# JuliaDSP/DSP.jl

Measured on NVIDIA H100. Metric: Gsamples/s filt+welch on 2^26 cplx-F32, higher is better.
Workload: dtype c64 (ComplexF32; f32 arithmetic)

## Files before the change

### __graft_entry__.py

```python
import os
import subprocess
import sys

ROOT = os.path.dirname(os.path.abspath(__file__))
PKG = os.path.join(ROOT, "dsp.jl_b200")


def build() -> None:
    jobs = str(min(8, os.cpu_count() or 2))
    subprocess.run(["make", "-C", os.path.join(PKG, "csrc"), "-j", jobs], check=True)
    host_dir = os.path.join(ROOT, "tests", "host")
    os.makedirs(os.path.join(ROOT, "build"), exist_ok=True)
    for name in ("fft_core_host_check", "fft_r32_host_check"):
        subprocess.run(["g++", "-std=c++17", "-O2", "-x", "c++", "-w", "-I/usr/local/cuda/include",
                        "-o", os.path.join(ROOT, "build", name), os.path.join(host_dir, name + ".cu")], check=True)
    for name in ("fir_tile_host_check", "fir_state_host_check"):
        subprocess.run(["g++", "-std=c++17", "-O2", "-march=native", "-x", "c++", "-w", "-I/usr/local/cuda/include",
                        "-o", os.path.join(ROOT, "build", name), os.path.join(host_dir, name + ".cu")], check=True)
    if ROOT not in sys.path:
        sys.path.insert(0, ROOT)
    import dspb200
    assert dspb200._lib.lib.dspb200_version() == 100


def smoke() -> None:
    if ROOT not in sys.path:
        sys.path.insert(0, ROOT)
    import numpy as np
    import dspb200
    from oracle import dspbase as od, periodograms as op, windows as ow

    if dspb200.device_count() < 1:
        raise RuntimeError("smoke() needs a CUDA device; dspb200 has no CPU fallback")
    rng = np.random.default_rng(7)
    x = (rng.standard_normal(1 << 16) + 1j * rng.standard_normal(1 << 16)).astype(np.complex64)
    v = (rng.standard_normal(513) + 1j * rng.standard_normal(513)).astype(np.complex64)
    y = dspb200.conv(x, v, algorithm="fft_overlapsave")
    ref = od.conv_exact(x, v)
    err = np.linalg.norm(y - ref) / np.linalg.norm(ref)
    assert y.dtype == np.complex64 and err < 1e-6, f"conv parity {err}"
    s = rng.standard_normal(1 << 18).astype(np.float32)
    p = dspb200.welch_pgram(s, 4096, 2048, window=dspb200.hanning)
    pref, _ = op.welch_pgram(s, 4096, 2048, window=ow.hanning, f64=True)
    err2 = np.linalg.norm(p.power - pref) / np.linalg.norm(pref)
    assert p.power.dtype == np.float32 and err2 < 1e-6, f"welch parity {err2}"
    print(f"smoke ok: conv relerr {err:.2e}, welch relerr {err2:.2e}, launches {dspb200.launch_count()}")


if __name__ == "__main__":
    build()
    if len(sys.argv) > 1 and sys.argv[1] == "smoke":
        smoke()
```

### dsp.jl_b200/csrc/fft_core.cuh

```cuda
#pragma once
#include "common.cuh"
#include <math.h>

#ifndef DSP_PROBE
#define DSP_PROBE 0
#endif

namespace dspb200 {

template <typename T> struct fft_pad { static constexpr int K = sizeof(T) == 4 ? 2 : 1; };
template <typename T> __host__ __device__ constexpr int fft_pad256(int n) {
    if (sizeof(T) == 4) return n == 512 ? 8 : (n == 1024 ? 4 : (n == 8192 ? 4 : 2));
    return n == 512 ? 4 : (n == 1024 ? 2 : (n == 8192 ? 2 : 1));
}
template <typename T> __host__ __device__ constexpr int fft_pad4096(int n) {
    if (sizeof(T) == 4) return n == 8192 ? 2 : (n == 16384 ? 4 : 0);
    return n == 8192 ? 1 : 0;
}
template <typename T, int N> __host__ __device__ __forceinline__ constexpr int padaddr(int p) {
    return p + fft_pad<T>::K * (p >> 4) + fft_pad256<T>(N) * (p >> 8) + fft_pad4096<T>(N) * (p >> 12);
}
template <typename T> __host__ __device__ constexpr int padded_len(int n) {
    return ((n - 1) + fft_pad<T>::K * ((n - 1) >> 4) + fft_pad256<T>(n) * ((n - 1) >> 8) + fft_pad4096<T>(n) * ((n - 1) >> 12) + 1 + 3) & ~3;
}
// ... 335 lines not shown
        fft_bfly<T, 16, false>(v0, w0);
#pragma unroll
        for (int r = 0; r < 16; ++r) p0[r * PS] = v0[r];
        fft_bfly<T, 16, false>(v1, w1);
#pragma unroll
        for (int r = 0; r < 16; ++r) p1[r * PS] = v1[r];
        return;
    }
#pragma unroll 1
    for (int it = 0; it < ITERS; ++it) {
        const int b = tid + it * NT;
        if (Q % NT != 0 && b >= Q) break;
        const int t = b & (S - 1);
        cx<T>* p = c.sm + padaddr<T, N>((b / S) * (16 * S) + t);
        cx<T> v[16], w[8];
        if constexpr (GATE && ITERS == 1) fft_gate_wait<NT>(tid);
        load_tw8<T, S, fft_tw_row(N)>(tab, t, w);
#pragma unroll
        for (int r = 0; r < 16; ++r) v[r] = p[r * PS];
        if constexpr (GATE && ITERS == 1) fft_gate_open<NT>(tid);
        fft_bfly<T, 16, false>(v, w);
#pragma unroll
        for (int r = 0; r < 16; ++r) p[r * PS] = v[r];
    }
}

template <typename T, int N, int NT, class Scope = FftCtaScope>
__device__ __forceinline__ void fft_middle(const FftCtx<T>& c, int tid, Scope sc = Scope()) {
    constexpr int NMID = fft_plan_traits<N>::NMID;
    static_assert(NMID < 2 || std::is_same<Scope, FftCtaScope>::value, "thread groups run transforms of at most 4096 points");
    if constexpr (NMID >= 1) {
#if !(DSP_PROBE & 16)
        fft_pass16<T, N, NT, 16, true>(c, tid);
#endif
        if constexpr (NMID == 2) {
            fft_group256_sync<NT>(tid);
#if !(DSP_PROBE & 1)
            fft_pass16<T, N, NT, 256>(c, tid);
#endif
        }
        sc.sync();
    }
}

template <typename T, int N>
__host__ __device__ __forceinline__ void fft_last_pass_load(const FftCtx<T>& c, int tp, cx<T> (&v)[16]) {
    constexpr int Q = fft_plan_traits<N>::Q;
    const cx<T>* p = c.sm + padaddr<T, N>(tp);
#pragma unroll
    for (int r = 0; r < 16; ++r) v[r] = p[padaddr<T, N>(r * Q)];
}
template <typename T, int N>
__host__ __device__ __forceinline__ void fft_last_pass_bfly(const FftCtx<T>& c, int tp, cx<T> (&v)[16]) {
    using P = fft_plan_traits<N>;
    constexpr int Q = P::Q, RL = P::RL;
    if constexpr (RL == 16) {
        cx<T> w[8];
        load_tw8<T, Q, fft_tw_row(N)>(Q == 16 ? c.t16 : c.t256, tp, w);
        fft_bfly<T, 16, false>(v, w);
    } else {
        constexpr int NBF = 16 / RL;
        constexpr int TLK = P::TLK;
#pragma unroll
        for (int a = 0; a < NBF; ++a) {
            const int t = tp + Q * a;
            cx<T> w[RL / 2];
            if constexpr (N == 16384) {
                const cx<T> w1 = fft_tl_in_smem<T, N>() ? c.tl[t] : ldtw<T>(c.tl, t);
                w[1] = w1;
                w[0] = mkc<T>(fma_(w1.x, w1.x, -(w1.y * w1.y)), (w1.x + w1.x) * w1.y);
            } else {
#pragma unroll
                for (int i = 0; i < TLK; ++i) w[i] = fft_tl_in_smem<T, N>() ? c.tl[t * TLK + i] : ldtw<T>(c.tl, t * TLK + i);
            }
            cx<T> u[RL];
#pragma unroll
            for (int j = 0; j < RL; ++j) u[j] = v[a + NBF * j];
            fft_bfly<T, RL, false>(u, w);
#pragma unroll
            for (int j = 0; j < RL; ++j) v[a + NBF * j] = u[j];
        }
    }
}
template <typename T, int N, int GATE_NT = 0>
__host__ __device__ __forceinline__ void fft_last_pass(const FftCtx<T>& c, int tp, cx<T> (&v)[16], int tid = 0) {
    if constexpr (GATE_NT > 256) fft_gate_wait<GATE_NT>(tid);
    fft_last_pass_load<T, N>(c, tp, v);
    if constexpr (GATE_NT > 256) fft_gate_open<GATE_NT>(tid);
    fft_last_pass_bfly<T, N>(c, tp, v);
}

template <int N> struct fft_last_chunks {
    static constexpr int RL = fft_plan_traits<N>::RL;
    static constexpr int COUNT = 16 / RL;
};
template <typename T, int N, int A>
__device__ __forceinline__ void fft_last_pass_chunk(const FftCtx<T>& c, int tp, cx<T> (&u)[fft_plan_traits<N>::RL]) {
    using P = fft_plan_traits<N>;
    constexpr int Q = P::Q, RL = P::RL, NBF = 16 / RL;
    const cx<T>* p = c.sm + padaddr<T, N>(tp);
#pragma unroll
    for (int j = 0; j < RL; ++j) u[j] = p[padaddr<T, N>((A + NBF * j) * Q)];
    if constexpr (RL == 16) {
        cx<T> w[8];
        load_tw8<T, Q, fft_tw_row(N)>(Q == 16 ? c.t16 : c.t256, tp, w);
        fft_bfly<T, 16, false>(u, w);
    } else {
        const int t = tp + Q * A;
        cx<T> w[RL / 2];
        if constexpr (N == 16384) {
            const cx<T> w1 = fft_tl_in_smem<T, N>() ? c.tl[t] : ldtw<T>(c.tl, t);
            w[1] = w1;
            w[0] = mkc<T>(fma_(w1.x, w1.x, -(w1.y * w1.y)), (w1.x + w1.x) * w1.y);
        } else {
#pragma unroll
            for (int i = 0; i < P::TLK; ++i) w[i] = fft_tl_in_smem<T, N>() ? c.tl[t * P::TLK + i] : ldtw<T>(c.tl, t * P::TLK + i);
        }
        fft_bfly<T, RL, false>(u, w);
    }
}

template <typename T, int N, int NT, class Ld0, class StLast>
__device__ __forceinline__ void fft_forward(const FftCtx<T>& c, int tid, Ld0 ld0, StLast stlast) {
    constexpr int Q = fft_plan_traits<N>::Q;
    constexpr int ITERS = (Q + NT - 1) / NT;
    fft_first_pass<T, N, NT, false>(c, tid, ld0);
    __syncthreads();
    fft_middle<T, N, NT>(c, tid);
#pragma unroll
    for (int it = 0; it < ITERS; ++it) {
        const int tp = tid + it * NT;
        if (Q % NT != 0 && tp >= Q) break;
        cx<T> v[16];
        fft_last_pass<T, N>(c, tp, v);
#pragma unroll
        for (int r = 0; r < 16; ++r) stlast(tp + r * Q, it, r, v[r]);
    }
}

struct fft_r32 {
    static constexpr int N = 16384;
    static constexpr int NT = 512;
    static constexpr int Q = N / 32;
    static constexpr int QL = N / 16;
    static constexpr int T32_LEN = 32 * 16;
    static constexpr int TL_LEN = 2 * QL;
    static constexpr int TABLE_LEN = T32_LEN + TL_LEN;
    static constexpr int C10 = 2;
    static constexpr int PADDED_LEN = ((N - 1) + C10 * ((N - 1) >> 10) + 1 + 3) & ~3;
    static constexpr int SMEM_ELEMS = PADDED_LEN + TABLE_LEN;
};
__host__ __device__ __forceinline__ constexpr int fft_r32_padaddr(int p) { return p + fft_r32::C10 * (p >> 10); }
__host__ __device__ __forceinline__ constexpr int fft_r32_block_of(int c) { return 32 * (c & 15) + (c >> 4); }

template <typename T> struct FftR32Ctx {
    cx<T>* sm;
    const cx<T>* t32;
    const cx<T>* tl;
};
template <typename T>
__device__ __forceinline__ FftR32Ctx<T> fft_r32_make_ctx(cx<T>* data, cx<T>* tabs, const cx<T>* __restrict__ g, int tid) {
    for (int i = tid; i < fft_r32::TABLE_LEN; i += fft_r32::NT) tabs[i] = g[i];
    return FftR32Ctx<T>{data, tabs, tabs + fft_r32::T32_LEN};
}

template <typename T> __host__ __device__ __forceinline__ void fft_r32_first_bfly(cx<T> (&v)[32]) { fft_bfly<T, 32, true>(v, nullptr); }
template <typename T> __host__ __device__ __forceinline__ void fft_r32_store_block(cx<T>* sm, int c, const cx<T> (&v)[32]) {
    cx<T>* p = sm + fft_r32_padaddr(32 * fft_r32_block_of(c));
#pragma unroll
    for (int r = 0; r < 32; r += 2) sts2<T>(p + r, v[r], v[r + 1]);
}

template <typename T, bool GATE = false> __host__ __device__ __forceinline__ void fft_r32_middle(const FftR32Ctx<T>& c, int tid) {
    const int t = tid & 31;
    cx<T>* p = c.sm + fft_r32_padaddr((tid >> 5) * 1024 + t);
    cx<T> v[32], w[16];
    if constexpr (GATE) fft_gate_wait<fft_r32::NT>(tid);
#pragma unroll
    for (int i = 0; i < 16; i += 2) lds2<T>(c.t32 + fft_tw_index<T>(i, t, 32), w[i], w[i + 1]);
#pragma unroll
    for (int r = 0; r < 32; ++r) v[r] = p[32 * r];
    if constexpr (GATE) fft_gate_open<fft_r32::NT>(tid);
    fft_bfly<T, 32, false>(v, w);
#pragma unroll
    for (int r = 0; r < 32; ++r) p[32 * r] = v[r];
}

template <typename T> __host__ __device__ __forceinline__ void fft_r32_last_load(const FftR32Ctx<T>& c, int t, cx<T> (&v)[16]) {
    const cx<T>* p = c.sm + fft_r32_padaddr(t);
#pragma unroll
    for (int s = 0; s < 16; ++s) v[s] = p[fft_r32_padaddr(s * 1024)];
}
template <typename T> __host__ __device__ __forceinline__ cx<T> fft_sq(cx<T> a) {
    return mkc<T>(fma_(a.x, a.x, -(a.y * a.y)), (a.x + a.x) * a.y);
}
template <typename T> __host__ __device__ __forceinline__ cx<T> fft_mul_const(cx<T> a, T cr, T ci) {
    return mkc<T>(fma_(a.x, cr, -(a.y * ci)), fma_(a.x, ci, a.y * cr));
}
template <typename T> __host__ __device__ __forceinline__ void fft_r32_last_bfly(const FftR32Ctx<T>& c, int t, cx<T> (&v)[16]) {
    const T c16 = fft_const<T>::C8, s16 = fft_const<T>::S8;
    cx<T> w[8];
    lds2<T>(c.tl + 2 * t, w[1], w[4]);
    w[2] = fft_sq(w[4]);
    w[0] = fft_sq(w[1]);
    w[3] = mul_w8<T>(w[2]);
    w[5] = fft_mul_const<T>(w[4], c16, -s16);
    w[6] = mul_w8<T>(w[4]);
    w[7] = fft_mul_const<T>(w[4], s16, -c16);
    fft_bfly<T, 16, false>(v, w);
}

template <typename T> inline void fft_fill_row(cx<T>* row, int R, long long num, long long den, int limit = 1 << 30) {
    const long double PI2 = 6.283185307179586476925286766559005768L;
    int qb = 0;
    for (int r = R; r > 1; r >>= 1) ++qb;
    int idx = 0;
    for (int k = 1; k <= qb; ++k) {
        const int cnt = k <= 2 ? 1 : (1 << (k - 2));
        for (int m = 0; m < cnt; ++m) {
            const long double a = -PI2 * ((long double)num * (long double)(R >> k) / (long double)den + (long double)m / (long double)(1 << k));
            if (idx < limit) row[idx] = mkc<T>((T)cosl(a), (T)sinl(a));
            ++idx;
        }
    }
}
template <typename T> inline void fft_fill_tables(cx<T>* t16, cx<T>* t256, long long n) {
    cx<T> row[8];
    const int nrow = fft_tw_row(n);
    const int keep6[6] = {0, 1, 2, 4, 5, 7};
    for (int t = 0; t < 16; ++t) {
        fft_fill_row<T>(row, 16, t, 256);
        for (int i = 0; i < nrow; ++i) t16[fft_tw_index<T>(i, t, 16)] = row[nrow == 8 ? i : keep6[i]];
    }
    for (int t = 0; t < 256; ++t) {
        fft_fill_row<T>(row, 16, t, 4096);
        for (int i = 0; i < nrow; ++i) t256[fft_tw_index<T>(i, t, 256)] = row[nrow == 8 ? i : keep6[i]];
    }
}
inline void fft_last_radix(long long n, int* rl, int* tlk) {
    int logn = 0;
    for (long long m = n; m > 1; m >>= 1) ++logn;
    const int ql = logn - 4;
    const int nmid = ql <= 4 ? 0 : (ql <= 8 ? 1 : 2);
    *rl = 1 << (ql - 4 * nmid);
    *tlk = *rl == 16 ? 0 : (n == 16384 ? 1 : *rl / 2);
}
inline long long fft_tl_len_rt(long long n) {
    int rl, tlk;
    fft_last_radix(n, &rl, &tlk);
    return (n / rl) * tlk;
}
template <typename T> inline void fft_fill_tl(cx<T>* tl, long long n) {
    int rl, tlk;
    fft_last_radix(n, &rl, &tlk);
    if (tlk == 0) return;
    const long double PI2 = 6.283185307179586476925286766559005768L;
    for (long long t = 0; t < n / rl; ++t) {
        if (n == 16384) {
            const long double a = -PI2 * (long double)t / (long double)n;
            tl[t] = mkc<T>((T)cosl(a), (T)sinl(a));
        } else {
            fft_fill_row<T>(tl + t * tlk, rl, t, n);
        }
    }
}

template <typename T> inline void fft_r32_fill_tables(cx<T>* tab) {
    cx<T> row[16];
    for (int t = 0; t < 32; ++t) {
        fft_fill_row<T>(row, 32, t, 1024);
        for (int i = 0; i < 16; ++i) tab[fft_tw_index<T>(i, t, 32)] = row[i];
    }
    const long double PI2 = 6.283185307179586476925286766559005768L;
    for (int t = 0; t < fft_r32::QL; ++t) {
        const long double a = -PI2 * (long double)t / (long double)fft_r32::N;
        tab[fft_r32::T32_LEN + 2 * t] = mkc<T>((T)cosl(4 * a), (T)sinl(4 * a));
        tab[fft_r32::T32_LEN + 2 * t + 1] = mkc<T>((T)cosl(a), (T)sinl(a));
    }
}

template <int N> struct fft_threads {
    static constexpr int NB16 = N / 16;
    static constexpr int value = NB16 < 64 ? 64 : (NB16 > 512 ? 512 : (NB16 > 256 ? 256 : NB16));
};
template <typename T, int N> struct fft_minblocks {
    static constexpr int value = sizeof(T) == 8 ? 1 : (fft_threads<N>::value >= 512 ? 1 : 512 / fft_threads<N>::value);
};

}
```

### dsp.jl_b200/csrc/overlap_save.cu

```cuda
#include "fft_core.cuh"
#include "async_copy.cuh"
#include "cufft_exec.cuh"
#include <math.h>
#include <stdlib.h>
#include <new>
#include <vector>

namespace dspb200 {

struct OsPlanImpl {
    int dtype = 0;
    bool cplx = false, f64 = false;
    int64_t nv = 0, nfft = 0, L = 0;
    bool fused = false;
    int device = 0;
    void* d_tw = nullptr;
    void* d_t16 = nullptr;
    void* d_t256 = nullptr;
    void* d_r32 = nullptr;
    int sm_count = 0;
    int fused_per_sm = 0;
    int fused_state_per_sm = 0;
    void* d_H = nullptr;
    cufftHandle fwd = 0, inv = 0;
    bool fft_ok = false;
    int64_t batch = 0, nbins = 0;
    DevBuf td, fd;
    HostPipe pipe;
};

template <typename T, bool CPLX> struct os_elt { using type = T; };
template <typename T> struct os_elt<T, true> { using type = cx<T>; };


template <typename T, int N, bool CPLX> struct os_threads {
    static constexpr bool f32 = sizeof(T) == 4;
    static constexpr int value = fft_threads<N>::value;
    static constexpr bool wide = f32 && ((N >= 512 && N <= 4096) || (N == 256 && !CPLX));
    static constexpr int minblocks = wide ? 1024 / value : fft_minblocks<T, N>::value;
    static constexpr bool staged = f32 && N == 16384;
};
constexpr int OS_STAGE_HEAD = 32768;
static_assert(OS_STAGE_HEAD % 16 == 0, "TMA copies move multiples of 16 bytes");
static_assert(OS_STAGE_HEAD < 16384 * 4, "the head region holds less than the shortest staged span (N + 1 floats)");
template <typename T, int N, bool CPLX> __host__ __device__ constexpr int os_fft_elems() {
    return os_threads<T, N, CPLX>::staged ? fft_r32::SMEM_ELEMS : fft_smem_elems<T, N>();
}
template <typename T, int N, bool CPLX> constexpr size_t os_smem_bytes() {
    return (size_t)os_fft_elems<T, N, CPLX>() * sizeof(cx<T>) + (os_threads<T, N, CPLX>::staged ? OS_STAGE_HEAD + 16 : 0);
}

template <typename T> __device__ __forceinline__ cx<T> ldg_cx(const cx<T>* __restrict__ p) {
    if constexpr (sizeof(T) == 4) {
        const float2 v = __ldg(reinterpret_cast<const float2*>(p));
        return mkc<T>(v.x, v.y);
    } else {
        const double2 v = __ldg(reinterpret_cast<const double2*>(p));
        return mkc<T>(v.x, v.y);
    }
}

template <typename E> struct OsUnit {
    const E* u;
    E* out;
    int jlo, jhi, jend, jzero;
    int nvm1, L;
};

template <typename E, bool STATE> struct OsState {};
template <typename E> struct OsState<E, true> {
    const E* si_in;
    E* si_out;
    int64_t nx;
};
template <typename E> struct OsUnitState {
    const E* si_in;
    E* si_out;
    int jsi, jnx;
};
struct OsNoState {};
template <typename E> __device__ __forceinline__ void os_put_state(const OsUnit<E>& g, const OsUnitState<E>& s, int j, E v) {
    if (j < s.jsi) v = v + s.si_in[j];
    if (j < s.jnx) g.out[j] = v;
    else s.si_out[j] = v;
}

__device__ __forceinline__ int os_clamp(int64_t v) {
    return (int)(v < -(int64_t(1) << 30) ? -(int64_t(1) << 30) : (v > (int64_t(1) << 30) ? (int64_t(1) << 30) : v));
}
__device__ __forceinline__ int os_clamp_diff(int64_t a, int64_t b) {
    return a >= (int64_t(1) << 62) ? (1 << 30) : os_clamp(a - b);
}

template <typename T, bool CPLX, bool INTERIOR>
__device__ __forceinline__ cx<T> os_sample(const OsUnit<typename os_elt<T, CPLX>::type>& g, int j) {
#if DSP_PROBE & 2
    return mkc<T>(T(j), T(1));
#endif
    if constexpr (CPLX) {
        if constexpr (INTERIOR) return g.u[j];
        return (j >= g.jlo && j < g.jhi) ? g.u[j] : mkc<T>(T(0), T(0));
    } else {
        const int jb = j + g.L;
        if constexpr (INTERIOR) return mkc<T>(g.u[j], g.u[jb]);
        const T a = (j >= g.jlo && j < g.jhi) ? g.u[j] : T(0);
        const T b = (jb >= g.jlo && jb < g.jhi) ? g.u[jb] : T(0);
        return mkc<T>(a, b);
    }
}

struct OsStage {
    unsigned char* head;
    uint64_t* bar;
    uint32_t bytes;
    uint32_t parity;
};

template <typename T, bool CPLX, bool INTERIOR, bool STATE, typename SGeom>
__device__ __forceinline__ void os_put(const OsUnit<typename os_elt<T, CPLX>::type>& g, const SGeom& sg, int j, cx<T> y) {
#if DSP_PROBE & 8
    if (y.x != T(123456.75)) return;
#endif
    if (j < g.nvm1) return;
    if constexpr (CPLX) {
        if constexpr (INTERIOR) g.out[j] = mkc<T>(y.y, y.x);
        else if constexpr (STATE) { if (j < g.jend) os_put_state(g, sg, j, mkc<T>(y.y, y.x)); }
        else if (j < g.jend) g.out[j] = (j < g.jzero) ? mkc<T>(y.y, y.x) : mkc<T>(T(0), T(0));
    } else {
        const int jb = j + g.L;
        if constexpr (INTERIOR) {
            g.out[j] = y.y;
            g.out[jb] = y.x;
        } else if constexpr (STATE) {
            if (j < g.jend) os_put_state(g, sg, j, y.y);
            if (jb < g.jend) os_put_state(g, sg, jb, y.x);
        } else {
            if (j < g.jend) g.out[j] = (j < g.jzero) ? y.y : T(0);
            if (jb < g.jend) g.out[jb] = (jb < g.jzero) ? y.x : T(0);
        }
    }
}
template <typename E, bool STATE, bool INTERIOR> using os_sgeom_t = std::conditional_t<STATE && !INTERIOR, OsUnitState<E>, OsNoState>;

template <typename T, int N, bool CPLX, int NT, bool INTERIOR, int ITERS, bool STATE, typename SG>
__device__ __forceinline__ void os_unit(const FftCtx<T>& ctx, int tid, const OsUnit<typename os_elt<T, CPLX>::type>& g,
                                        const cx<T>* __restrict__ H, const SG& state_geometry) {
    using E = typename os_elt<T, CPLX>::type;
    constexpr int Q = fft_plan_traits<N>::Q;
    static_assert(ITERS == (Q + NT - 1) / NT, "register tile does not match the thread count");
    {
        auto ld0 = [&](int j, int, int) -> cx<T> { return os_sample<T, CPLX, INTERIOR>(g, j); };
        fft_first_pass<T, N, NT, true>(ctx, tid, ld0);
    }
    __syncthreads();
    fft_middle<T, N, NT>(ctx, tid);
    cx<T> v[ITERS][16];
#pragma unroll
    for (int it = 0; it < ITERS; ++it) {
        const int tp = tid + it * NT;
        if (Q % NT == 0 || tp < Q) {
            fft_last_pass<T, N, (ITERS == 1 && Q % NT == 0) ? NT : 0>(ctx, tp, v[it], tid);
#pragma unroll
#if DSP_PROBE & 4
            for (int r = 0; r < 16; ++r) v[it][r] = cswap(cmul(v[it][r], mkc<T>(T(0.5), T(r))));
#else
            for (int r = 0; r < 16; ++r) v[it][r] = cswap(cmul(v[it][r], ldg_cx<T>(H + tp + r * Q)));
#endif
            fft_bfly16_plain<T>(v[it]);
        }
    }
    __syncthreads();
#pragma unroll
    for (int it = 0; it < ITERS; ++it) {
        const int tp = tid + it * NT;
        if (Q % NT == 0 || tp < Q) fft_store_block<T, N>(ctx.sm, tp, v[it]);
    }
    __syncthreads();
    fft_middle<T, N, NT>(ctx, tid);
    constexpr int RL = fft_plan_traits<N>::RL, NBF = 16 / RL;
    os_sgeom_t<E, STATE, INTERIOR> sg{};
    if constexpr (STATE && !INTERIOR) sg = state_geometry();
    auto chunk = [&](auto a_, int tp) {
        constexpr int A = decltype(a_)::value;
        cx<T> u[RL];
        fft_last_pass_chunk<T, N, A>(ctx, tp, u);
#pragma unroll
        for (int jj = 0; jj < RL; ++jj) os_put<T, CPLX, INTERIOR, STATE>(g, sg, tp + (A + NBF * jj) * Q, u[jj]);
    };
#pragma unroll
    for (int it = 0; it < ITERS; ++it) {
        const int tp = tid + it * NT;
        if (Q % NT != 0 && tp >= Q) break;
        chunk(std::integral_constant<int, 0>{}, tp);
        if constexpr (NBF >= 2) chunk(std::integral_constant<int, 1>{}, tp);
        if constexpr (NBF >= 4) { chunk(std::integral_constant<int, 2>{}, tp); chunk(std::integral_constant<int, 3>{}, tp); }
        if constexpr (NBF >= 8) {
            chunk(std::integral_constant<int, 4>{}, tp); chunk(std::integral_constant<int, 5>{}, tp);
            chunk(std::integral_constant<int, 6>{}, tp); chunk(std::integral_constant<int, 7>{}, tp);
        }
    }
}

template <typename T, bool CPLX, bool INTERIOR, bool STATE, typename SG>
__device__ __forceinline__ void os_unit_r32(const FftR32Ctx<T>& ctx, int tid, const OsUnit<typename os_elt<T, CPLX>::type>& g,
                                            const cx<T>* __restrict__ H, OsStage& st, bool staged,
                                            const typename os_elt<T, CPLX>::type* __restrict__ next_u, const SG& state_geometry) {
    using E = typename os_elt<T, CPLX>::type;
    constexpr int NT = fft_r32::NT, Q = fft_r32::Q;
    cx<T> v[32];
    if (INTERIOR && staged) {
        mbar_wait(st.bar, st.parity);
        st.parity ^= 1;
        const E* s = reinterpret_cast<const E*>(st.head);
#pragma unroll
        for (int m = 0; m < 32; ++m) {
            const int j = tid + m * Q;
            if constexpr (CPLX) v[m] = s[j];
            else v[m] = mkc<T>(s[j], s[j + g.L]);
        }
    } else {
#pragma unroll
        for (int m = 0; m < 32; ++m) v[m] = os_sample<T, CPLX, INTERIOR>(g, tid + m * Q);
    }
    fft_r32_first_bfly<T>(v);
    __syncthreads();
    fft_r32_store_block<T>(ctx.sm, tid, v);
    __syncthreads();
    if (next_u != nullptr && tid == 0) {
        fence_proxy_async_shared();
        mbar_expect_tx_noarrive(st.bar, OS_STAGE_HEAD);
        tma_load_1d(st.head, next_u, OS_STAGE_HEAD, st.bar);
    }
#if !(DSP_PROBE & 16)
    fft_r32_middle<T, true>(ctx, tid);
#endif
    __syncthreads();
    {
        cx<T> u[2][16];
#pragma unroll
        for (int it = 0; it < 2; ++it) {
            fft_r32_last_load<T>(ctx, tid + it * NT, u[it]);
            fft_r32_last_bfly<T>(ctx, tid + it * NT, u[it]);
        }
#pragma unroll
#if DSP_PROBE & 4
        for (int m = 0; m < 32; ++m) v[m] = cswap(cmul(u[m & 1][m >> 1], mkc<T>(T(0.5), T(m))));
#else
        for (int m = 0; m < 32; ++m) v[m] = cswap(cmul(u[m & 1][m >> 1], ldg_cx<T>(H + tid + m * Q)));
#endif
    }
    fft_r32_first_bfly<T>(v);
    __syncthreads();
    fft_r32_store_block<T>(ctx.sm, tid, v);
    __syncthreads();
#if !(DSP_PROBE & 16)
    fft_r32_middle<T, true>(ctx, tid);
#endif
    __syncthreads();
    os_sgeom_t<E, STATE, INTERIOR> sg{};
    if constexpr (STATE && !INTERIOR) sg = state_geometry();
    cx<T> w[2][16];
#pragma unroll
    for (int it = 0; it < 2; ++it) fft_r32_last_load<T>(ctx, tid + it * NT, w[it]);
    if (next_u != nullptr) {
        __syncthreads();
        if (tid == 0) {
            fence_proxy_async_shared();
            mbar_expect_tx(st.bar, st.bytes - OS_STAGE_HEAD);
            tma_load_1d(ctx.sm, reinterpret_cast<const unsigned char*>(next_u) + OS_STAGE_HEAD, st.bytes - OS_STAGE_HEAD, st.bar);
        }
    }
#pragma unroll
    for (int it = 0; it < 2; ++it) {
        const int t = tid + it * NT;
        fft_r32_last_bfly<T>(ctx, t, w[it]);
#pragma unroll
        for (int s = 0; s < 16; ++s) os_put<T, CPLX, INTERIOR, STATE>(g, sg, t + s * fft_r32::QL, w[it][s]);
    }
}

template <typename T, int N, bool CPLX, bool STATE>
__global__ void __launch_bounds__((os_threads<T, N, CPLX>::value), (os_threads<T, N, CPLX>::minblocks))
os_fused_kernel(const void* __restrict__ u_, int64_t u_begin, int64_t nu_local, int64_t u_col_stride,
                void* __restrict__ out_, int64_t out_begin, int64_t out_count, int64_t out_col_stride,
                int64_t zero_from, int nv, int64_t units_per_col, int64_t total_units, const cx<T>* __restrict__ gtl,
                const cx<T>* __restrict__ g16, const cx<T>* __restrict__ g256, const cx<T>* __restrict__ H,
                const OsState<typename os_elt<T, CPLX>::type, STATE> sa) {
    constexpr int NT = os_threads<T, N, CPLX>::value;
    constexpr int Q = fft_plan_traits<N>::Q;
    constexpr int ITERS = (Q + NT - 1) / NT;
    constexpr bool STAGED = os_threads<T, N, CPLX>::staged;
    extern __shared__ __align__(16) unsigned char smem_raw[];
    constexpr int HEAD = STAGED ? OS_STAGE_HEAD : 0;
    cx<T>* sm = reinterpret_cast<cx<T>*>(smem_raw + HEAD);
    using E = typename os_elt<T, CPLX>::type;
    const int tid = threadIdx.x;
    pdl_launch_dependents();
    auto make_ctx = [&]() {
        if constexpr (STAGED) return fft_r32_make_ctx<T>(sm, sm + fft_r32::PADDED_LEN, gtl, tid);
        else return fft_make_ctx<T, N, NT>(sm, g16, g256, gtl, tid);
    };
    const auto ctx = make_ctx();
    OsStage st;
    st.head = smem_raw;
    st.bar = reinterpret_cast<uint64_t*>(smem_raw + HEAD + (size_t)os_fft_elems<T, N, CPLX>() * sizeof(cx<T>));
    st.parity = 0;
    if constexpr (STAGED) {
        if (tid == 0) {
            mbar_init(st.bar, 1);
            mbar_fence_init();
        }
    }
    pdl_wait();
    __syncthreads();
    const int L = N - nv + 1;
    const int span = CPLX ? N : N + L;
    st.bytes = (uint32_t)((span * sizeof(E) + 15) & ~(size_t)15);

    const bool onecol = units_per_col >= total_units;
    auto geometry = [&](int64_t gu, OsUnit<E>& g) -> bool {
        const int64_t col = onecol ? 0 : gu / units_per_col;
        const int64_t unit = gu - col * units_per_col;
        const int64_t q = CPLX ? unit : 2 * unit;
        const int64_t s0 = out_begin + q * L - (nv - 1);
        const int64_t i0 = s0 - u_begin;
        g.u = reinterpret_cast<const E*>(u_) + col * u_col_stride + i0;
        g.out = reinterpret_cast<E*>(out_) + col * out_col_stride + (s0 - out_begin);
        g.jlo = os_clamp(-i0);
        g.jhi = os_clamp(nu_local - i0);
        g.jend = os_clamp(out_begin + out_count - s0);
        g.jzero = os_clamp_diff(zero_from, s0);
        g.nvm1 = nv - 1;
        g.L = L;
        return g.jlo <= 0 && g.jhi >= span && g.jend >= span && g.jzero >= span;
    };
    auto state_geometry = [&](int64_t gu) {
        OsUnitState<E> s{};
        if constexpr (STATE) {
            const int64_t col = onecol ? 0 : gu / units_per_col;
            const int64_t unit = gu - col * units_per_col;
            const int64_t s0 = out_begin + (CPLX ? unit : 2 * unit) * L - (nv - 1);
            s.si_in = sa.si_in + col * (nv - 1) + s0;
            s.si_out = sa.si_out + col * (nv - 1) + (s0 - sa.nx);
            s.jsi = sa.si_in ? os_clamp((nv - 1) - s0) : -(1 << 30);
            s.jnx = os_clamp(sa.nx - s0);
        }
        return s;
    };
    auto l2_prefetch = [&](int64_t gn) {
        if (tid == 0 && gn < total_units) {
            const int64_t coln = onecol ? 0 : gn / units_per_col;
            const int64_t qn = (CPLX ? 1 : 2) * (gn - coln * units_per_col);
            int64_t lo = out_begin + qn * L - (nv - 1) - u_begin;
            int64_t hi = lo + span;
            if (lo < 0) lo = 0;
            if (hi > nu_local) hi = nu_local;
            const uintptr_t a0 = ((uintptr_t)(reinterpret_cast<const E*>(u_) + coln * u_col_stride + lo) + 15) & ~(uintptr_t)15;
            const uintptr_t a1 = (uintptr_t)(reinterpret_cast<const E*>(u_) + coln * u_col_stride + hi) & ~(uintptr_t)15;
            if (hi > lo && a1 > a0) tma_prefetch_l2(reinterpret_cast<const void*>(a0), (uint32_t)(a1 - a0));
        }
    };
    auto stage_src = [&](int64_t gn) -> const E* {
        if (!STAGED || gn >= total_units || (DSP_PROBE & 2)) return nullptr;
        OsUnit<E> gl;
        if (!geometry(gn, gl)) return nullptr;
        if ((int64_t)gl.jhi * (int64_t)sizeof(E) < (int64_t)st.bytes || ((uintptr_t)gl.u & 15) != 0) return nullptr;
        return gl.u;
    };
    bool staged = false;
    if constexpr (STAGED) {
        const E* src = stage_src(blockIdx.x);
        staged = src != nullptr;
        if (staged && tid == 0) {
            mbar_expect_tx(st.bar, st.bytes);
            tma_load_1d(st.head, src, OS_STAGE_HEAD, st.bar);
            tma_load_1d(ctx.sm, reinterpret_cast<const unsigned char*>(src) + OS_STAGE_HEAD, st.bytes - OS_STAGE_HEAD, st.bar);
        }
    }

    for (int64_t gu = blockIdx.x; gu < total_units; gu += gridDim.x) {
        l2_prefetch(gu + (int64_t)gridDim.x);
        OsUnit<E> g;
        const bool interior = geometry(gu, g);
        const E* next_u = stage_src(gu + gridDim.x);
        auto sgeom = [&]() { return state_geometry(gu); };
        if constexpr (STAGED) {
            if (interior) os_unit_r32<T, CPLX, true, STATE>(ctx, tid, g, H, st, staged, next_u, sgeom);
            else os_unit_r32<T, CPLX, false, STATE>(ctx, tid, g, H, st, staged, next_u, sgeom);
        } else {
            if (interior) os_unit<T, N, CPLX, NT, true, ITERS, STATE>(ctx, tid, g, H, sgeom);
            else os_unit<T, N, CPLX, NT, false, ITERS, STATE>(ctx, tid, g, H, sgeom);
        }
        staged = next_u != nullptr;
    }
}

template <typename T, int N, bool CPLX>
__global__ void __launch_bounds__(fft_threads<N>::value, fft_minblocks<T, N>::value)
os_filter_kernel(const void* __restrict__ v_, int nv, const cx<T>* __restrict__ gtl, const cx<T>* __restrict__ g16,
                 const cx<T>* __restrict__ g256, cx<T>* __restrict__ H) {
    constexpr int NT = fft_threads<N>::value;
    extern __shared__ __align__(16) unsigned char smem_raw[];
    cx<T>* sm = reinterpret_cast<cx<T>*>(smem_raw);
    using E = typename os_elt<T, CPLX>::type;
    const E* v = reinterpret_cast<const E*>(v_);
    const FftCtx<T> ctx = fft_make_ctx<T, N, NT>(sm, g16, g256, gtl, threadIdx.x);
    __syncthreads();
    const T scale = T(1) / T(N);
    auto ld0 = [&](int j, int, int) -> cx<T> {
        if (j >= nv) return mkc<T>(T(0), T(0));
        if constexpr (CPLX) return v[j]; else return mkc<T>(v[j], T(0));
    };
    auto stl = [&](int k, int, int, cx<T> x) { H[k] = cscale(x, scale); };
    fft_forward<T, N, NT>(ctx, threadIdx.x, ld0, stl);
}

template <typename T, bool CPLX>
__global__ void os_gather_kernel(const void* __restrict__ u_, int64_t u_begin, int64_t nu_local, int64_t m_first,
                                 int64_t L, int64_t nv, int64_t nfft, int64_t nblk, void* __restrict__ td_) {
    using E = typename os_elt<T, CPLX>::type;
    const E* u = reinterpret_cast<const E*>(u_);
    E* td = reinterpret_cast<E*>(td_);
    const int64_t total = nblk * nfft;
    for (int64_t i = (int64_t)blockIdx.x * blockDim.x + threadIdx.x; i < total; i += (int64_t)gridDim.x * blockDim.x) {
        const int64_t b = i / nfft, j = i - b * nfft;
        const int64_t src = m_first + b * L - (nv - 1) + j - u_begin;
        E v;
        if constexpr (CPLX) v = mkc<T>(T(0), T(0)); else v = T(0);
        if (src >= 0 && src < nu_local) v = u[src];
        td[i] = v;
    }
}

template <typename T>
__global__ void os_cmul_kernel(cx<T>* __restrict__ X, const cx<T>* __restrict__ H, int64_t nbins, int64_t nblk) {
    const int64_t total = nblk * nbins;
    for (int64_t i = (int64_t)blockIdx.x * blockDim.x + threadIdx.x; i < total; i += (int64_t)gridDim.x * blockDim.x)
        X[i] = cmul(X[i], H[i % nbins]);
}

template <typename T>
__global__ void hilbert_weight_kernel(cx<T>* __restrict__ X, int64_t n, int64_t ncols, T scale) {
    const int64_t total = n * ncols;
    const int64_t last2 = (n + 1) / 2 - 1;
    for (int64_t i = (int64_t)blockIdx.x * blockDim.x + threadIdx.x; i < total; i += (int64_t)gridDim.x * blockDim.x) {
        const int64_t k = i % n;
        if (k > n / 2) { X[i] = mkc<T>(T(0), T(0)); continue; }
        const T w = (k >= 1 && k <= last2) ? T(2) * scale : scale;
        X[i] = cscale(X[i], w);
    }
}

struct Dims3 { int64_t n[3]; };

template <typename E>
__global__ void nd_copy_kernel(const E* __restrict__ src, Dims3 s, E* __restrict__ dst, Dims3 d, E zero) {
    const int64_t total = d.n[0] * d.n[1] * d.n[2];
    for (int64_t i = (int64_t)blockIdx.x * blockDim.x + threadIdx.x; i < total; i += (int64_t)gridDim.x * blockDim.x) {
        const int64_t i0 = i % d.n[0], i1 = (i / d.n[0]) % d.n[1], i2 = i / (d.n[0] * d.n[1]);
        dst[i] = (i0 < s.n[0] && i1 < s.n[1] && i2 < s.n[2]) ? src[i0 + s.n[0] * (i1 + s.n[1] * i2)] : zero;
    }
}

template <typename T, bool CPLX, bool RANK1>
__global__ void conv_direct_nd_kernel(const void* __restrict__ u_, Dims3 su, const void* __restrict__ v_, Dims3 sv,
                                      void* __restrict__ out_) {
    using E = typename os_elt<T, CPLX>::type;
    const bool walk_u = su.n[0] <= sv.n[0];
    const E* w = reinterpret_cast<const E*>(walk_u ? u_ : v_);
    const E* o = reinterpret_cast<const E*>(walk_u ? v_ : u_);
    const Dims3 sw = walk_u ? su : sv, so = walk_u ? sv : su;
    E* out = reinterpret_cast<E*>(out_);
    const int64_t o0 = su.n[0] + sv.n[0] - 1, o1 = su.n[1] + sv.n[1] - 1, o2 = su.n[2] + sv.n[2] - 1;
    const int64_t total = o0 * o1 * o2;
    for (int64_t i = (int64_t)blockIdx.x * blockDim.x + threadIdx.x; i < total; i += (int64_t)gridDim.x * blockDim.x) {
        const int64_t k0 = RANK1 ? i : i % o0, k1 = RANK1 ? 0 : (i / o0) % o1, k2 = RANK1 ? 0 : i / (o0 * o1);
        T ar = T(0), ai = T(0);
        for (int64_t m2 = max(k2 - (so.n[2] - 1), (int64_t)0); m2 <= min(k2, sw.n[2] - 1); ++m2)
            for (int64_t m1 = max(k1 - (so.n[1] - 1), (int64_t)0); m1 <= min(k1, sw.n[1] - 1); ++m1)
                for (int64_t m0 = max(k0 - (so.n[0] - 1), (int64_t)0); m0 <= min(k0, sw.n[0] - 1); ++m0) {
                    const E p = w[m0 + sw.n[0] * (m1 + sw.n[1] * m2)];
                    const E q = o[(k0 - m0) + so.n[0] * ((k1 - m1) + so.n[1] * (k2 - m2))];
                    const E a = walk_u ? p : q, b = walk_u ? q : p;
                    if constexpr (CPLX) {
                        ar = fma(a.x, b.x, fma(-a.y, b.y, ar));
                        ai = fma(a.x, b.y, fma(a.y, b.x, ai));
                    } else {
                        ar = fma(a, b, ar);
                    }
                }
        if constexpr (CPLX) out[i] = mkc<T>(ar, ai); else out[i] = ar;
    }
}

struct OsNd { int64_t su[3], sv[3], so[3], nf[3], L[3], nb[3]; };

template <typename E>
__global__ void nd_os_gather_kernel(const E* __restrict__ u, OsNd g, int64_t blk0, int64_t nblk, E* __restrict__ td, E zero) {
    const int64_t per = g.nf[0] * g.nf[1] * g.nf[2], total = per * nblk, nblocks = g.nb[0] * g.nb[1] * g.nb[2];
    for (int64_t i = (int64_t)blockIdx.x * blockDim.x + threadIdx.x; i < total; i += (int64_t)gridDim.x * blockDim.x) {
        const int64_t b = blk0 + i / per, r = i % per;
        E val = zero;
        if (b < nblocks) {
            const int64_t i0 = r % g.nf[0], i1 = (r / g.nf[0]) % g.nf[1], i2 = r / (g.nf[0] * g.nf[1]);
            const int64_t b0 = b % g.nb[0], b1 = (b / g.nb[0]) % g.nb[1], b2 = b / (g.nb[0] * g.nb[1]);
            const int64_t s0 = g.L[0] * b0 - (g.sv[0] - 1) + i0, s1 = g.L[1] * b1 - (g.sv[1] - 1) + i1,
                          s2 = g.L[2] * b2 - (g.sv[2] - 1) + i2;
            if (s0 >= 0 && s0 < g.su[0] && s1 >= 0 && s1 < g.su[1] && s2 >= 0 && s2 < g.su[2])
                val = u[s0 + g.su[0] * (s1 + g.su[1] * s2)];
        }
        td[i] = val;
    }
}

template <typename E>
__global__ void nd_os_scatter_kernel(const E* __restrict__ td, OsNd g, int64_t blk0, int64_t nblk, E* __restrict__ out) {
    const int64_t per = g.L[0] * g.L[1] * g.L[2], total = per * nblk, nblocks = g.nb[0] * g.nb[1] * g.nb[2];
    const int64_t nfp = g.nf[0] * g.nf[1] * g.nf[2];
    for (int64_t i = (int64_t)blockIdx.x * blockDim.x + threadIdx.x; i < total; i += (int64_t)gridDim.x * blockDim.x) {
        const int64_t lb = i / per, b = blk0 + lb, r = i % per;
        if (b >= nblocks) continue;
        const int64_t j0 = r % g.L[0], j1 = (r / g.L[0]) % g.L[1], j2 = r / (g.L[0] * g.L[1]);
        const int64_t b0 = b % g.nb[0], b1 = (b / g.nb[0]) % g.nb[1], b2 = b / (g.nb[0] * g.nb[1]);
        const int64_t o0 = g.L[0] * b0 + j0, o1 = g.L[1] * b1 + j1, o2 = g.L[2] * b2 + j2;
        if (o0 < g.so[0] && o1 < g.so[1] && o2 < g.so[2])
            out[o0 + g.so[0] * (o1 + g.so[1] * o2)] =
                td[lb * nfp + (j0 + g.sv[0] - 1) + g.nf[0] * ((j1 + g.sv[1] - 1) + g.nf[1] * (j2 + g.sv[2] - 1))];
    }
}

template <typename T, bool CPLX, bool STATE>
__global__ void os_scatter_kernel(const void* __restrict__ td_, int64_t m_first, int64_t L, int64_t nv, int64_t nfft,
                                  int64_t nblk, void* __restrict__ out_, int64_t out_begin, int64_t out_end,
                                  int64_t zero_from, const OsState<typename os_elt<T, CPLX>::type, STATE> sa) {
    using E = typename os_elt<T, CPLX>::type;
    const E* td = reinterpret_cast<const E*>(td_);
    E* out = reinterpret_cast<E*>(out_);
    const int64_t total = nblk * L;
    for (int64_t i = (int64_t)blockIdx.x * blockDim.x + threadIdx.x; i < total; i += (int64_t)gridDim.x * blockDim.x) {
        const int64_t b = i / L, j = i - b * L;
        const int64_t m = m_first + b * L + j;
        if (m < out_end) {
            E v = td[b * nfft + (nv - 1) + j];
            if (m >= zero_from) { if constexpr (CPLX) v = mkc<T>(T(0), T(0)); else v = T(0); }
            if constexpr (STATE) {
                if (sa.si_in && m < nv - 1) v = v + sa.si_in[m];
                if (m >= sa.nx) {
                    sa.si_out[m - sa.nx] = v;
                    continue;
                }
            }
            out[m - out_begin] = v;
        }
    }
}

template <typename T, bool CPLX>
__global__ void pad_copy_kernel(const void* __restrict__ src_, int64_t n, void* __restrict__ dst_, int64_t nfft, T scale) {
    using E = typename os_elt<T, CPLX>::type;
    const E* src = reinterpret_cast<const E*>(src_);
    E* dst = reinterpret_cast<E*>(dst_);
    for (int64_t i = (int64_t)blockIdx.x * blockDim.x + threadIdx.x; i < nfft; i += (int64_t)gridDim.x * blockDim.x) {
        E v;
        if constexpr (CPLX) v = mkc<T>(T(0), T(0)); else v = T(0);
        if (i < n) {
            v = src[i];
// ... 591 lines not shown
```

Before: 76.14.

## Restructure staged 16384-point FFT convolution to keep spectrum in permuted order

Reworks the staged overlap-save forward FFT into a decimation-in-frequency pass: a radix-16 butterfly with twiddles in registers, then warp-local radix-32 column and row passes. The spectrum stays in a permuted order, so the filter spectrum H is stored with a matching index permutation. The inverse FFT then starts directly from registers. This drops one full shared-memory round trip and several block-wide barriers per block, replacing some with __syncwarp, and uses a new stride-32 padded layout. In exchange there is more twiddle arithmetic, and padding changes that could cause bank conflicts.

```diff
diff --git a/__graft_entry__.py b/__graft_entry__.py
--- a/__graft_entry__.py
+++ b/__graft_entry__.py
@@ -11,7 +11,7 @@
     subprocess.run(["make", "-C", os.path.join(PKG, "csrc"), "-j", jobs], check=True)
     host_dir = os.path.join(ROOT, "tests", "host")
     os.makedirs(os.path.join(ROOT, "build"), exist_ok=True)
-    for name in ("fft_core_host_check", "fft_r32_host_check"):
+    for name in ("fft_core_host_check", "fft_r32_host_check", "fft_r32w_host_check"):
         subprocess.run(["g++", "-std=c++17", "-O2", "-x", "c++", "-w", "-I/usr/local/cuda/include",
                         "-o", os.path.join(ROOT, "build", name), os.path.join(host_dir, name + ".cu")], check=True)
     for name in ("fir_tile_host_check", "fir_state_host_check"):
diff --git a/dsp.jl_b200/csrc/fft_core.cuh b/dsp.jl_b200/csrc/fft_core.cuh
--- a/dsp.jl_b200/csrc/fft_core.cuh
+++ b/dsp.jl_b200/csrc/fft_core.cuh
@@ -511,6 +511,15 @@
 };
 __host__ __device__ __forceinline__ constexpr int fft_r32_padaddr(int p) { return p + fft_r32::C10 * (p >> 10); }
 __host__ __device__ __forceinline__ constexpr int fft_r32_block_of(int c) { return 32 * (c & 15) + (c >> 4); }
+struct fft_r32_lay10 {
+    static constexpr int PADDED_LEN = fft_r32::PADDED_LEN;
+    __host__ __device__ static constexpr int addr(int p) { return fft_r32_padaddr(p); }
+};
+struct fft_r32_lay5 {
+    static constexpr int C5 = 2;
+    static constexpr int PADDED_LEN = fft_r32::N + C5 * (fft_r32::N >> 5);
+    __host__ __device__ static constexpr int addr(int p) { return p + C5 * (p >> 5); }
+};
 
 template <typename T> struct FftR32Ctx {
     cx<T>* sm;
@@ -524,31 +533,34 @@
 }
 
 template <typename T> __host__ __device__ __forceinline__ void fft_r32_first_bfly(cx<T> (&v)[32]) { fft_bfly<T, 32, true>(v, nullptr); }
-template <typename T> __host__ __device__ __forceinline__ void fft_r32_store_block(cx<T>* sm, int c, const cx<T> (&v)[32]) {
-    cx<T>* p = sm + fft_r32_padaddr(32 * fft_r32_block_of(c));
+template <typename T, class Lay = fft_r32_lay10>
+__host__ __device__ __forceinline__ void fft_r32_store_block(cx<T>* sm, int c, const cx<T> (&v)[32]) {
+    cx<T>* p = sm + Lay::addr(32 * fft_r32_block_of(c));
 #pragma unroll
     for (int r = 0; r < 32; r += 2) sts2<T>(p + r, v[r], v[r + 1]);
 }
 
-template <typename T, bool GATE = false> __host__ __device__ __forceinline__ void fft_r32_middle(const FftR32Ctx<T>& c, int tid) {
+template <typename T, bool GATE = false, class Lay = fft_r32_lay10>
+__host__ __device__ __forceinline__ void fft_r32_middle(const FftR32Ctx<T>& c, int tid) {
     const int t = tid & 31;
-    cx<T>* p = c.sm + fft_r32_padaddr((tid >> 5) * 1024 + t);
+    cx<T>* p = c.sm + Lay::addr((tid >> 5) * 1024 + t);
     cx<T> v[32], w[16];
     if constexpr (GATE) fft_gate_wait<fft_r32::NT>(tid);
 #pragma unroll
     for (int i = 0; i < 16; i += 2) lds2<T>(c.t32 + fft_tw_index<T>(i, t, 32), w[i], w[i + 1]);
 #pragma unroll
-    for (int r = 0; r < 32; ++r) v[r] = p[32 * r];
+    for (int r = 0; r < 32; ++r) v[r] = p[Lay::addr(32 * r)];
     if constexpr (GATE) fft_gate_open<fft_r32::NT>(tid);
     fft_bfly<T, 32, false>(v, w);
 #pragma unroll
-    for (int r = 0; r < 32; ++r) p[32 * r] = v[r];
-}
-
-template <typename T> __host__ __device__ __forceinline__ void fft_r32_last_load(const FftR32Ctx<T>& c, int t, cx<T> (&v)[16]) {
-    const cx<T>* p = c.sm + fft_r32_padaddr(t);
-#pragma unroll
-    for (int s = 0; s < 16; ++s) v[s] = p[fft_r32_padaddr(s * 1024)];
+    for (int r = 0; r < 32; ++r) p[Lay::addr(32 * r)] = v[r];
+}
+
+template <typename T, class Lay = fft_r32_lay10>
+__host__ __device__ __forceinline__ void fft_r32_last_load(const FftR32Ctx<T>& c, int t, cx<T> (&v)[16]) {
+    const cx<T>* p = c.sm + Lay::addr(t);
+#pragma unroll
+    for (int s = 0; s < 16; ++s) v[s] = p[Lay::addr(s * 1024)];
 }
 template <typename T> __host__ __device__ __forceinline__ cx<T> fft_sq(cx<T> a) {
     return mkc<T>(fma_(a.x, a.x, -(a.y * a.y)), (a.x + a.x) * a.y);
@@ -567,6 +579,53 @@
     w[6] = mul_w8<T>(w[4]);
     w[7] = fft_mul_const<T>(w[4], s16, -c16);
     fft_bfly<T, 16, false>(v, w);
+}
+
+struct fft_r32w {
+    using Lay = fft_r32_lay5;
+    static constexpr int SMEM_ELEMS = Lay::PADDED_LEN + fft_r32::TABLE_LEN;
+};
+__host__ __device__ __forceinline__ constexpr int fft_r32w_hidx(int k) { return (k & ~511) | ((k & 15) << 5) | ((k >> 4) & 31); }
+
+template <typename T> __host__ __device__ __forceinline__ void fft_r32w_dif16(const FftR32Ctx<T>& c, int n2, cx<T> (&u)[16]) {
+    fft_bfly<T, 16, true>(u, nullptr);
+    cx<T> wb[4], wa[4];
+    lds2<T>(c.tl + 2 * n2, wa[1], wb[1]);
+    wb[2] = fft_sq(wb[1]);
+    wb[3] = cmul(wb[2], wb[1]);
+    wa[2] = fft_sq(wa[1]);
+    wa[3] = cmul(wa[2], wa[1]);
+#pragma unroll
+    for (int b = 1; b < 4; ++b) u[b] = cmul(u[b], wb[b]);
+#pragma unroll
+    for (int a = 1; a < 4; ++a) {
+        u[4 * a] = cmul(u[4 * a], wa[a]);
+#pragma unroll
+        for (int b = 1; b < 4; ++b) u[4 * a + b] = cmul(u[4 * a + b], cmul(wa[a], wb[b]));
+    }
+}
+template <typename T> __host__ __device__ __forceinline__ void fft_r32w_store16(cx<T>* sm, int n2, const cx<T> (&u)[16]) {
+    cx<T>* p = sm + fft_r32_lay5::addr(n2);
+#pragma unroll
+    for (int k = 0; k < 16; ++k) p[fft_r32_lay5::addr(1024 * k)] = u[k];
+}
+template <typename T> __host__ __device__ __forceinline__ void fft_r32w_col(cx<T>* sm, int g, int l) {
+    cx<T>* p = sm + fft_r32_lay5::addr(1024 * g + l);
+    cx<T> v[32];
+#pragma unroll
+    for (int r = 0; r < 32; ++r) v[r] = p[fft_r32_lay5::addr(32 * r)];
+    fft_bfly<T, 32, true>(v, nullptr);
+#pragma unroll
+    for (int r = 0; r < 32; ++r) p[fft_r32_lay5::addr(32 * r)] = v[r];
+}
+template <typename T> __host__ __device__ __forceinline__ void fft_r32w_row(const FftR32Ctx<T>& c, int g, int l, cx<T> (&v)[32]) {
+    const cx<T>* p = c.sm + fft_r32_lay5::addr(1024 * g + 32 * l);
+    cx<T> w[16];
+#pragma unroll
+    for (int i = 0; i < 16; i += 2) lds2<T>(c.t32 + fft_tw_index<T>(i, l, 32), w[i], w[i + 1]);
+#pragma unroll
+    for (int r = 0; r < 32; r += 2) lds2<T>(p + r, v[r], v[r + 1]);
+    fft_bfly<T, 32, false>(v, w);
 }
 
 template <typename T> inline void fft_fill_row(cx<T>* row, int R, long long num, long long den, int limit = 1 << 30) {
diff --git a/dsp.jl_b200/csrc/overlap_save.cu b/dsp.jl_b200/csrc/overlap_save.cu
--- a/dsp.jl_b200/csrc/overlap_save.cu
+++ b/dsp.jl_b200/csrc/overlap_save.cu
@@ -44,7 +44,7 @@
 static_assert(OS_STAGE_HEAD % 16 == 0, "TMA copies move multiples of 16 bytes");
 static_assert(OS_STAGE_HEAD < 16384 * 4, "the head region holds less than the shortest staged span (N + 1 floats)");
 template <typename T, int N, bool CPLX> __host__ __device__ constexpr int os_fft_elems() {
-    return os_threads<T, N, CPLX>::staged ? fft_r32::SMEM_ELEMS : fft_smem_elems<T, N>();
+    return os_threads<T, N, CPLX>::staged ? fft_r32w::SMEM_ELEMS : fft_smem_elems<T, N>();
 }
 template <typename T, int N, bool CPLX> constexpr size_t os_smem_bytes() {
     return (size_t)os_fft_elems<T, N, CPLX>() * sizeof(cx<T>) + (os_threads<T, N, CPLX>::staged ? OS_STAGE_HEAD + 16 : 0);
@@ -206,7 +206,9 @@
                                             const cx<T>* __restrict__ H, OsStage& st, bool staged,
                                             const typename os_elt<T, CPLX>::type* __restrict__ next_u, const SG& state_geometry) {
     using E = typename os_elt<T, CPLX>::type;
+    using Lay = fft_r32w::Lay;
     constexpr int NT = fft_r32::NT, Q = fft_r32::Q;
+    const int k1 = tid >> 5, l = tid & 31;
     cx<T> v[32];
     if (INTERIOR && staged) {
         mbar_wait(st.bar, st.parity);
@@ -222,46 +224,52 @@
 #pragma unroll
         for (int m = 0; m < 32; ++m) v[m] = os_sample<T, CPLX, INTERIOR>(g, tid + m * Q);
     }
-    fft_r32_first_bfly<T>(v);
-    __syncthreads();
-    fft_r32_store_block<T>(ctx.sm, tid, v);
+#pragma unroll
+    for (int it = 0; it < 2; ++it) {
+        cx<T> u[16];
+#pragma unroll
+        for (int n1 = 0; n1 < 16; ++n1) u[n1] = v[2 * n1 + it];
+        fft_r32w_dif16<T>(ctx, tid + it * NT, u);
+#pragma unroll
+        for (int k = 0; k < 16; ++k) v[2 * k + it] = u[k];
+    }
     __syncthreads();
     if (next_u != nullptr && tid == 0) {
         fence_proxy_async_shared();
         mbar_expect_tx_noarrive(st.bar, OS_STAGE_HEAD);
         tma_load_1d(st.head, next_u, OS_STAGE_HEAD, st.bar);
     }
-#if !(DSP_PROBE & 16)
-    fft_r32_middle<T, true>(ctx, tid);
-#endif
-    __syncthreads();
-    {
-        cx<T> u[2][16];
-#pragma unroll
-        for (int it = 0; it < 2; ++it) {
-            fft_r32_last_load<T>(ctx, tid + it * NT, u[it]);
-            fft_r32_last_bfly<T>(ctx, tid + it * NT, u[it]);
-        }
-#pragma unroll
-#if DSP_PROBE & 4
-        for (int m = 0; m < 32; ++m) v[m] = cswap(cmul(u[m & 1][m >> 1], mkc<T>(T(0.5), T(m))));
-#else
-        for (int m = 0; m < 32; ++m) v[m] = cswap(cmul(u[m & 1][m >> 1], ldg_cx<T>(H + tid + m * Q)));
-#endif
-    }
-    fft_r32_first_bfly<T>(v);
-    __syncthreads();
-    fft_r32_store_block<T>(ctx.sm, tid, v);
+#pragma unroll
+    for (int it = 0; it < 2; ++it) {
+        cx<T> u[16];
+#pragma unroll
+        for (int k = 0; k < 16; ++k) u[k] = v[2 * k + it];
+        fft_r32w_store16<T>(ctx.sm, tid + it * NT, u);
+    }
     __syncthreads();
 #if !(DSP_PROBE & 16)
-    fft_r32_middle<T, true>(ctx, tid);
+    fft_r32w_col<T>(ctx.sm, k1, l);
+    __syncwarp();
+#endif
+    fft_r32w_row<T>(ctx, k1, l, v);
+#pragma unroll
+#if DSP_PROBE & 4
+    for (int m = 0; m < 32; ++m) v[m] = cswap(cmul(v[m], mkc<T>(T(0.5), T(m))));
+#else
+    for (int m = 0; m < 32; ++m) v[m] = cswap(cmul(v[m], ldg_cx<T>(H + tid + m * Q)));
+#endif
+    fft_r32_first_bfly<T>(v);
+    fft_r32_store_block<T, Lay>(ctx.sm, k1 + 16 * l, v);
+    __syncwarp();
+#if !(DSP_PROBE & 16)
+    fft_r32_middle<T, false, Lay>(ctx, tid);
 #endif
     __syncthreads();
     os_sgeom_t<E, STATE, INTERIOR> sg{};
     if constexpr (STATE && !INTERIOR) sg = state_geometry();
     cx<T> w[2][16];
 #pragma unroll
-    for (int it = 0; it < 2; ++it) fft_r32_last_load<T>(ctx, tid + it * NT, w[it]);
+    for (int it = 0; it < 2; ++it) fft_r32_last_load<T, Lay>(ctx, tid + it * NT, w[it]);
     if (next_u != nullptr) {
         __syncthreads();
         if (tid == 0) {
@@ -297,7 +305,7 @@
     const int tid = threadIdx.x;
     pdl_launch_dependents();
     auto make_ctx = [&]() {
-        if constexpr (STAGED) return fft_r32_make_ctx<T>(sm, sm + fft_r32::PADDED_LEN, gtl, tid);
+        if constexpr (STAGED) return fft_r32_make_ctx<T>(sm, sm + fft_r32w::Lay::PADDED_LEN, gtl, tid);
         else return fft_make_ctx<T, N, NT>(sm, g16, g256, gtl, tid);
     };
     const auto ctx = make_ctx();
@@ -411,7 +419,7 @@
         if (j >= nv) return mkc<T>(T(0), T(0));
         if constexpr (CPLX) return v[j]; else return mkc<T>(v[j], T(0));
     };
-    auto stl = [&](int k, int, int, cx<T> x) { H[k] = cscale(x, scale); };
+    auto stl = [&](int k, int, int, cx<T> x) { H[os_threads<T, N, CPLX>::staged ? fft_r32w_hidx(k) : k] = cscale(x, scale); };
     fft_forward<T, N, NT>(ctx, threadIdx.x, ld0, stl);
 }
 
```

Measured after the change: 76.51 (median of 6 runs). No clear change (+0.5%).
